# DaehwanKimLab/centrifuge

Measured on AMD Instinct MI355X. Metric: classified reads/sec (whole node) on 100bp synthetic reads vs p_compressed; HBM GB/s achieved, higher is better.
Workload: dtype u64

## Files before the change

### centrifuge_amd/csrc/cf_device.hip

```cpp
#include <hip/hip_runtime.h>
#include <sched.h>
#include <dlfcn.h>

#include <algorithm>
#include <cmath>
#include <chrono>
#include <cstdio>
#include <cstdlib>
#include <cstring>
#include <memory>
#include <mutex>
#include <stdexcept>
#include <string>
#include <vector>

#include "../../include/centrifuge_amd.h"
#include "cf_index.hpp"
#include "cf_kernels.hpp"
#include "cf_scan.hpp"
#include "cf_textio.hpp"
#include "cf_inflate.hpp"
#include "cf_restore.hpp"
#include "cf_plan.hpp"
#include "cf_knobs.hpp"
// ... 47 lines not shown
__global__ void __launch_bounds__(256) k_search(DIndex ix, DParams pr, DBatch b) { search_body<G>(ix, pr, b); }

__global__ void __launch_bounds__(256) k_rlen(const uint64_t *off, uint32_t *rlen, uint32_t nReads) { rlen_body(off, rlen, nReads, cf_global_thread()); }
__global__ void __launch_bounds__(256) k_convert(DConvert c) { convert_body(c, cf_global_thread()); }
__global__ void __launch_bounds__(256) k_dense_unpack(DUnpack u) { dense_unpack_body(u, (uint64_t)blockIdx.x * blockDim.x + threadIdx.x); }
__global__ void __launch_bounds__(256) k_pack(DBatch b, uint8_t *recs, uint32_t W) { pack_body(b, recs, W, cf_global_thread()); }

template <int G, int W, bool COUNT>
__global__ void __launch_bounds__(256) __attribute__((amdgpu_waves_per_eu(COUNT ? 1 : W == 4 ? 6 : W == 6 ? 5 : 4, 8))) k_search2(DIndex ix, DParams pr, DBatch b) {
    __shared__ __attribute__((aligned(16))) uint8_t lds[(256 / G) * rec_lds_stride(W) + 256 * 4 * RankTab<G>::WORDS + (256 / G) * 16 * kLazyHits];
    search2_body<G, W, COUNT>(ix, pr, b, lds);
}

template <int W, bool COUNT, int LZ = 0, bool MULTI = false>
__global__ void __launch_bounds__(256) __attribute__((amdgpu_waves_per_eu((W == 4 && LZ == 1) ? 7 : (W == 4 && MULTI) ? 6 : (W == 6 && MULTI) ? 5 : 1, 8))) k_search2_l1(DIndex ix, DParams pr, DBatch b) {
    __shared__ __attribute__((aligned(16))) uint8_t lds[256 * rec_lds_stride(W) + 256 * 16 * (LZ ? LZ : (int)lazy_hits(1, W))];
    search2_body<1, W, COUNT, true, LZ, MULTI>(ix, pr, b, lds);
}
__global__ void __launch_bounds__(256) k_pair_planes(DIndex ix, uint8_t *planes2, uint64_t nGroups) {
    pair_planes_body(ix, planes2, (uint64_t)blockIdx.x * blockDim.x + threadIdx.x, nGroups);
}
__global__ void __launch_bounds__(256) k_occ_planes(DIndex ix, uint8_t *planes, uint64_t nSides) {
    occ_planes_body(ix, planes, (uint64_t)blockIdx.x * blockDim.x + threadIdx.x, nSides);
}
__global__ void __launch_bounds__(256) k_repeat_probe(DIndex ix, uint32_t nSamples, uint32_t depth, uint32_t *hits) {
    const uint32_t i = cf_global_thread();
    bool yes = false;
    if (i < nSamples && ix.len > 2) {
        uint64_t x = 0x9e3779b97f4a7c15ull * (i + 1);
        x ^= x >> 29; x *= 0xbf58476d1ce4e5b9ull; x ^= x >> 32;
        yes = repeat_probe_body(ix, x % (ix.len - 1), depth);
    }
    const uint64_t m = cf_ballot(yes);
    if (m && cf_lane() == (uint32_t)cf_ctz64(m)) (void)cf_atomic_add(hits, (uint32_t)cf_popc64(m));
}

__global__ void __launch_bounds__(256) k_post_fast(DIndex ix, DParams pr, DBatch b) {
    const uint32_t q = cf_global_thread();
    const bool d = q < b.nQueries ? post_fast_body(ix, pr, b, q) : false;
    if (q < b.nQueries && b.postDeferred) b.postDeferred[q] = d ? 1 : 0;
    defer_push(b.slowPost, &b.st->nSlowPost, d, q);
}
template <bool EARLY>
__global__ void __launch_bounds__(256) k_score_fast(DIndex ix, DParams pr, DBatch b) {
    const uint32_t q = cf_global_thread();
    const bool d = q < b.nQueries ? score_fast_body<EARLY>(ix, pr, b, q) : false;
    defer_push(b.slowScore, &b.st->nSlowScore, d, q);
}
__global__ void __launch_bounds__(256) k_list_all(uint32_t *list, uint32_t *counter, uint32_t n) {
    const uint32_t q = cf_global_thread();
    if (q < n) list[q] = q;
    if (q == 0) *counter = n;
}
__global__ void __launch_bounds__(64) __attribute__((amdgpu_waves_per_eu(3, 8))) k_post(DIndex ix, DParams pr, DBatch b, uint32_t capHits) {
    extern __shared__ __attribute__((aligned(16))) uint8_t ldsPost[];
    HitP *scratch = capHits ? reinterpret_cast<HitP *>(ldsPost) + (size_t)cf_local_thread() * capHits : nullptr;
    const uint32_t n = b.st->nSlowPost;
    for (uint32_t i = cf_global_thread(); i < n; i += cf_global_threads()) post_body(ix, pr, b, b.slowPost[i], scratch, capHits);
}
__global__ void __launch_bounds__(64) k_postfix_only(DIndex ix, DParams pr, DBatch b) {
    const uint32_t i = cf_global_thread();
    if (i < b.st->nItems / 2) post_fix(ix, pr, b, b.items[i]);
}
__global__ void k_window(DBatch b, uint32_t qLo, bool keepSlow) { if (cf_global_thread() == 0) row_window_body(b, qLo, keepSlow); }
__global__ void __launch_bounds__(256) k_emit(DParams pr, DBatch b) {
    const uint32_t q = cf_global_thread();
    if (q < b.nQueries) emit_body(pr, b, q);
}
template <int G, bool COUNT>
__global__ void __launch_bounds__(256) k_walk2(DIndex ix, DBatch b) { walk2_body<G, COUNT>(ix, b); }
template <int MODE>
__global__ void __launch_bounds__(256) k_walk_table(DIndex ix, DBatch b) { walk2_body<2, false, MODE>(ix, b); }
template <typename T>
__global__ void __launch_bounds__(256) k_stop_samples(DIndex ix, T *stopVal, uint64_t *stopBits, uint64_t nSamples) {
    for (uint64_t i = (uint64_t)blockIdx.x * blockDim.x + threadIdx.x; i < nSamples; i += (uint64_t)gridDim.x * blockDim.x) {
        const uint64_t pos = trio_at(ix.saPos, i << ix.offRate);
        stopVal[pos] = static_cast<const T *>(ix.offs)[i];
        cf_atomic_or64(&stopBits[pos >> 6], 1ull << (pos & 63));
    }
}
template <typename T>
__global__ void __launch_bounds__(256) k_stop_bounds(DIndex ix, T *stopVal, uint64_t *stopBits) {
    for (uint64_t j = (uint64_t)blockIdx.x * blockDim.x + threadIdx.x; j < ix.nBound; j += (uint64_t)gridDim.x * blockDim.x) {
        const uint64_t pos = trio_at(ix.saPos, ix.boundRow[j]);
        stopVal[pos] = (T)ix.boundRef[j];
        cf_atomic_or64(&stopBits[pos >> 6], 1ull << (pos & 63));
    }
}
template <typename T>
__global__ void k_stop_end(DIndex ix, T *stopVal, uint64_t *stopBits) {
    const uint64_t pos = trio_at(ix.saPos, ix.zOff);
    stopVal[pos] = 0;
    cf_atomic_or64(&stopBits[pos >> 6], 1ull << (pos & 63));
}
template <typename T>
__global__ void __launch_bounds__(256) k_table_by_position(DIndex ix, const T *stopVal, const uint64_t *stopBits, T *table, uint64_t nRows, uint32_t *walkMax) {
    uint32_t gap = 0;
    for (uint64_t row = (uint64_t)blockIdx.x * blockDim.x + threadIdx.x; row < nRows; row += (uint64_t)gridDim.x * blockDim.x) {
        const uint64_t pos = trio_at(ix.saPos, row);
        uint64_t w = pos >> 6;
        uint64_t m = stopBits[w] & (~0ull >> (63 - (pos & 63)));
        while (m == 0 && w > 0) m = stopBits[--w];
        const uint64_t pred = m ? (w << 6) + 63 - (uint64_t)__builtin_clzll(m) : 0;
        table[row] = stopVal[pred];
        const uint32_t g = (uint32_t)(pos - pred);
        gap = g > gap ? g : gap;
    }
    for (int d = 32; d > 0; d >>= 1) { const uint32_t o = __shfl_xor(gap, d, 64); gap = o > gap ? o : gap; }
    if ((threadIdx.x & 63) == 0 && gap) atomicMax(walkMax, gap);
}
template <typename T>
// ... 1199 lines not shown
    d.recs = bt->recWords && !bt->selfRecords ? bt->recs.p : nullptr; d.recWords = bt->recWords;
    d.itemMeta = bt->selfRecords ? bt->itemMeta.p : nullptr;
}

static void enqueuePlan(cf_batch *bt, hipStream_t st) {
    const uint64_t nReads = bt->nReads;
    const DPlan &pl = bt->pl;
    HIP_OK(hipStreamWaitEvent(st, bt->ev[8], 0));
    if (bt->densePending) {
        const uint32_t L = bt->densePending - 1;
        const DUnpack u{bt->dense.p, bt->bases.p, bt->rlen.p, (uint32_t)nReads, L, bt->revDelta ? bt->bases.p + bt->revDelta : nullptr};
        bt->revMade = bt->revDelta != 0;
        const uint64_t threads = nReads * std::max<uint64_t>(((uint64_t)L + 31) >> 5, 1);
        hipLaunchKernelGGL(k_dense_unpack, dim3((unsigned)((threads + 255) / 256)), dim3(256), 0, st, u);
        bt->densePending = 0;
    }
    HIP_OK(hipEventRecord(bt->ev[5], st));
    HIP_OK(hipMemsetAsync(bt->st.p, 0, sizeof(BatchStatus), st));
    const dim3 gp((unsigned)((nReads + 1 + 255) / 256)), bl(256);
    if (bt->fromBytes && nReads) hipLaunchKernelGGL(k_rlen, gp, bl, 0, st, bt->off8.p, bt->rlen.p, (uint32_t)nReads);
    scan_enqueue<SCAN_WORDS>(bt->rlen.p, nReads, bt->woff.p, nullptr, bt->tileA.p, bt->tileC.p, st);
    if (bt->fromBytes && nReads) {
        DConvert c{bt->seq.p, bt->off8.p, bt->woff.p, bt->bases.p, bt->nmask.p, (uint32_t)nReads};
        hipLaunchKernelGGL(k_convert, dim3((unsigned)((nReads + 255) / 256)), dim3(256), 0, st, c);
    }
    if (bt->fromText && nReads) {
        const DTextPack c{bt->text.p, bt->txSeqOff.p, bt->rlen.p, bt->woff.p, bt->bases.p, bt->nmask.p, (uint32_t)nReads};
        hipLaunchKernelGGL(k_text_pack, dim3((unsigned)((nReads + 255) / 256)), dim3(256), 0, st, c);
    }
    hipLaunchKernelGGL(k_plan, gp, bl, 0, st, pl);
    scan_enqueue<SCAN_HITS>(bt->hitCap.p, nReads, bt->hitBase.p, bt->slotOf.p, bt->tileA.p, bt->tileC.p, st);
    hipLaunchKernelGGL(k_plan_fill, gp, bl, 0, st, pl);
    if (pl.revDelta && nReads && !bt->revMade) {
        const uint64_t threads = nReads * (uint64_t)bt->recWords;
        hipLaunchKernelGGL(k_rev_words, dim3((unsigned)((threads + 255) / 256)), bl, 0, st, pl, bt->recWords);
    }
    if (bt->nQueries) hipLaunchKernelGGL(k_plan_maxscore, dim3((unsigned)((bt->nQueries + 255) / 256)), bl, 0, st, bt->rlen.p, bt->pass.p,
                                         (uint32_t)bt->nQueries, bt->paired, bt->maxScore.p);
    if (bt->recWords && !bt->selfRecords && nReads) {
        const uint64_t threads = 2 * nReads * (uint64_t)bt->recWords;
        hipLaunchKernelGGL(k_pack, dim3((unsigned)((threads + 255) / 256)), bl, 0, st, bt->d, bt->recs.p, bt->recWords);
    }
    HIP_OK(hipEventRecord(bt->ev[6], st));
    bt->planned = true;
}

static dim3 listGrid(const cf_index &ix, uint64_t nq) { return dim3((unsigned)std::max<uint64_t>(1, std::min<uint64_t>((nq + 63) / 64, (uint64_t)ix.numCUs * 32))); }

static bool earlyScoreMode(const cf_batch *bt) {
    static const bool on = envInt("CF_EARLY_SCORE", 0) != 0 && envInt("CF_POST_FAST", 1) != 0 && envInt("CF_SCORE_FAST", 1) != 0 && envInt("CF_TAIL_STREAM", 0) == 0;
    return on && bt->d.directRefs != 0 && bt->tail != nullptr && bt->nQueries != 0;
}

static void enqueuePost(cf_batch *bt, hipStream_t st) {
    cf_classifier *cl = bt->cl;
    cf_index &ix = *cl->ix;
    const DBatch &d = bt->d;
    const uint32_t nq = (uint32_t)bt->nQueries;
    if (!nq) return;
    static const bool fast = envInt("CF_POST_FAST", 1) != 0;
    if (fast) hipLaunchKernelGGL(k_post_fast, dim3((nq + 255) / 256), dim3(256), 0, st, ix.d, cl->d, d);
    else hipLaunchKernelGGL(k_list_all, dim3((nq + 255) / 256), dim3(256), 0, st, bt->slowPost.p, &bt->st.p->nSlowPost, nq);
    if (earlyScoreMode(bt)) {
        HIP_OK(hipEventRecord(bt->evPostFast, st));
        HIP_OK(hipStreamWaitEvent(bt->tail, bt->evPostFast, 0));
        hipLaunchKernelGGL(k_post, listGrid(ix, nq), dim3(64), 0, bt->tail, ix.d, cl->d, d, 0u);
        HIP_OK(hipEventRecord(bt->evPost, bt->tail));
        hipLaunchKernelGGL(k_score_fast<true>, dim3((nq + 255) / 256), dim3(256), 0, st, ix.d, cl->d, d);
        HIP_OK(hipStreamWaitEvent(st, bt->evPost, 0));
        return;
    }
    static const bool postLds = envInt("CF_POST_LDS", 0) != 0;
    const uint32_t capHits = postLds ? (uint32_t)std::min<uint64_t>(60, 2 * ((uint64_t)bt->maxLenHost / (uint64_t)std::max(1, ix.h.g.ftabChars) + 2)) : 0u;
    hipLaunchKernelGGL(k_post, listGrid(ix, nq), dim3(64), (size_t)64 * capHits * sizeof(HitP), st, ix.d, cl->d, d, capHits);
}

static bool enqueueRowPass(cf_batch *bt, uint32_t qLo, hipStream_t st, bool marks, hipStream_t late = nullptr, bool early = false) {
    cf_classifier *cl = bt->cl;
    cf_index &ix = *cl->ix;
    const DBatch &d = bt->d;
    const uint32_t nq = (uint32_t)bt->nQueries;
    static const bool fast = envInt("CF_SCORE_FAST", 1) != 0;
    HIP_OK(hipMemsetAsync(bt->cursor.p + 1, 0, 8, st));
    hipLaunchKernelGGL(k_window, dim3(1), dim3(64), 0, st, d, qLo, early);
    const bool direct = d.directRefs != 0;
    if (nq && !direct) hipLaunchKernelGGL(k_emit, dim3((nq + 255) / 256), dim3(256), 0, st, cl->d, d);
    if (marks) HIP_OK(hipEventRecord(bt->ev[2], st));
    const bool counted = nq && !direct ? launchWalk(cl, bt, st) : true;
    if (marks) HIP_OK(hipEventRecord(bt->ev[3], st));
    if (nq) {
        if (early) {}
        else if (fast) hipLaunchKernelGGL(k_score_fast<false>, dim3((nq + 255) / 256), dim3(256), 0, st, ix.d, cl->d, d);
        else hipLaunchKernelGGL(k_list_all, dim3((nq + 255) / 256), dim3(256), 0, st, bt->slowScore.p, &bt->st.p->nSlowScore, nq);
        if (late && late != st) {
            HIP_OK(hipEventRecord(bt->evLate, st));
            HIP_OK(hipStreamWaitEvent(late, bt->evLate, 0));
            st = late;
        }
        if (direct) hipLaunchKernelGGL(k_resolve_slow, listGrid(ix, nq), dim3(64), 0, st, ix.d, cl->d, d);
        static const uint32_t capRows = (uint32_t)std::clamp(envInt("CF_SCORE_LDS_ROWS", 0), 0, 64), sparse = (uint32_t)std::clamp(envInt("CF_SCORE_LDS_SPARSE", 2), 1, 64);
        hipLaunchKernelGGL(k_score, listGrid(ix, nq), dim3(64), (size_t)(64 / sparse) * score_scratch_bytes(capRows), st, ix.d, cl->d, d, capRows, capRows ? sparse : 1u, 0u, 0xffffffffu);
        static const uint32_t slotBits = (uint32_t)std::clamp(envInt("CF_COUNT_SLOT_BITS", (int)kCountSlotBits), 1, (int)kCountSlotBits);
        hipLaunchKernelGGL(k_count, dim3((nq + kCountChunk - 1) / kCountChunk), dim3(1024), 0, st, d, slotBits, d.nTaxa <= (1u << slotBits));
    }
    if (marks) HIP_OK(hipEventRecord(bt->ev[4], st));
    return counted;
}

static void enqueueCompact(cf_batch *bt, hipStream_t st) {
    const uint32_t nq = (uint32_t)bt->nQueries;
    const dim3 g((nq + 1 + 255) / 256), bl(256);
    scan_enqueue<SCAN_PLAIN>(bt->nOut.p, nq, bt->rowFirst.p, nullptr, bt->tileA.p, bt->tileC.p, st);
    const bool narrow = bt->resultFormat == CF_RESULTS_NARROW;
    const DCompact c{bt->out.p, bt->o1tax.p, bt->o1a.p, bt->o1b.p, bt->d.oStride, bt->nOut.p, bt->rowFirst.p, (uint32_t)bt->cl->d.k, nq, bt->outCompact.p, bt->st.p,
                     narrow ? reinterpret_cast<NarrowRow *>(bt->outCompact.p) : nullptr, bt->qinfo.p, bt->pass.p, bt->paired};
    hipLaunchKernelGGL(k_compact, g, bl, 0, st, c);
}

static void enqueueClassify(cf_batch *bt, hipStream_t st) {
    cf_classifier *cl = bt->cl;
    HIP_OK(hipMemsetAsync(bt->cursor.p, 0, 32, st));
    HIP_OK(hipMemsetAsync(bt->ops.p, 0, sizeof(OpCounts), st));
    static const bool allFast = envInt("CF_POST_FAST", 1) != 0 && envInt("CF_SCORE_FAST", 1) != 0;
    if (!allFast) {
        HIP_OK(hipMemsetAsync(bt->qRows.p, 0, 4 * (bt->nQueries + 1), st));
        HIP_OK(hipMemsetAsync(bt->nOut.p, 0, 4 * (bt->nQueries + 1), st));
    }
// ... 1303 lines not shown
```

### centrifuge_amd/csrc/cf_kernels.hpp

```cpp
#pragma once
#include "cf_platform.hpp"

namespace cfamd {

constexpr uint32_t kNone32 = 0xffffffffu;
constexpr uint64_t kNone64 = ~0ull;
constexpr uint32_t kSideChars = 384;
constexpr int kSearchChunk = CF_WAVE;

struct RefInfo { uint64_t tax; uint32_t tidx, pid; };
static_assert(sizeof(RefInfo) == 16, "RefInfo layout");
struct DIndex {
    const uint8_t *sides;
    const uint64_t *ftab, *eftab;
    uint64_t fchr0, fchr1, fchr2, fchr3;
    uint64_t len, zOff, zSide;
    uint32_t zIn;
    int32_t ftabChars, offRate, offw;
    const void *offs;
    const uint8_t *planes;
    const uint8_t *planes2;
    const uint64_t *wide;
    int32_t wideChars;
    const uint64_t *text;
// ... 1633 lines not shown
    bool tried = false;
    uint32_t run = 0;
    while (dep < L) {
        if (ix.posRate >= 0 && !tried && bot - top == 1 && run >= ix.verifyMinRun && (top & ((1ull << ix.posRate) - 1)) == 0 &&
            L - dep >= kVerifyMinLeft) {
            tried = true;
            const uint64_t p = trio_at(ix.saPos, top >> ix.posRate);
            uint64_t tw = 0, twi = kNone64;
            uint32_t M = 0;
            while (dep + M < L && M < p) {
                const uint64_t pos = p - 1 - M;
                if ((pos >> 5) != twi) { twi = pos >> 5; tw = ix.text[twi]; }
                const int rc = strand_char(b, wbase, L, fw, L - (dep + M) - 1, win);
                if (rc > 3 || (uint64_t)rc != ((tw >> (2 * (pos & 31))) & 3)) break;
                M++;
            }
            const uint64_t pe = p - M, pm = (1ull << ix.isaRate) - 1, q = (pe + pm) & ~pm;
            if ((b.lazyHits & 4u) && (dep + M >= L || M < p)) {
                h.top = kRowIsPos | pe; h.bot = h.top + 1; h.len = dep + M - cur;
                return;
            }
            if (M >= 4 && M >= q - pe) {
                dep = dep + M - (uint32_t)(q - pe);
                top = trio_at(ix.isa, q >> ix.isaRate); bot = top + 1;
                continue;
            }
        }
        const int c = strand_char(b, wbase, L, fw, L - dep - 1, win);
        if (c > 3) break;
        uint64_t t, bb;
        { bool two; rank_any<G>(ix, c, top, bot, t, bb, two); }
        if (bb <= t) break;
        run = (bb - t == 1 && bot - top == 1) ? run + 1 : 0;
        top = t; bot = bb; dep++;
    }
    h.top = top; h.bot = bot; h.len = dep - cur;
}

CF_DEV bool hit_less(const HitP &a, const HitP &b) {
    const uint64_t as = hp_size(a), bs = hp_size(b);
    const uint64_t al = hp_len(a), bl = hp_len(b);
    if (al >= 22 || bl >= 22) {
        if (al >= 22 && bl >= 22) { if (as < bs) return true; if (as > bs) return false; }
        if (bl < al) return true;
        if (bl > al) return false;
    }
    if (bl * as < al * bs) return true;
    if (bl * as > al * bs) return false;
    if (as < bs) return true;
    if (as > bs) return false;
    if (bl < al) return true;
    return false;
}
CF_DEV void hit_swap(HitP &a, HitP &b) { const HitP t = a; a = b; b = t; }

CF_DEV void ss_linear_insert(HitP *a, int last) {
    const HitP val = a[last];
    int next = last - 1;
    while (hit_less(val, a[next])) { a[last] = a[next]; last = next; --next; }
    a[last] = val;
}
CF_DEV void ss_insertion(HitP *a, int first, int last) {
    if (first == last) return;
    for (int i = first + 1; i != last; ++i) {
        if (hit_less(a[i], a[first])) {
            const HitP val = a[i];
            for (int k = i; k > first; --k) a[k] = a[k - 1];
            a[first] = val;
        } else ss_linear_insert(a, i);
    }
}
CF_DEV void ss_push_heap(HitP *a, int first, int hole, int top, const HitP &val) {
    int parent = (hole - 1) / 2;
    while (hole > top && hit_less(a[first + parent], val)) {
        a[first + hole] = a[first + parent]; hole = parent; parent = (hole - 1) / 2;
    }
    a[first + hole] = val;
}
CF_DEV void ss_adjust_heap(HitP *a, int first, int hole, int len, const HitP &val) {
    const int top = hole;
    int child = hole;
    while (child < (len - 1) / 2) {
        child = 2 * (child + 1);
        if (hit_less(a[first + child], a[first + (child - 1)])) child--;
        a[first + hole] = a[first + child]; hole = child;
    }
    if ((len & 1) == 0 && child == (len - 2) / 2) {
        child = 2 * (child + 1);
        a[first + hole] = a[first + (child - 1)]; hole = child - 1;
    }
    ss_push_heap(a, first, hole, top, val);
}
CF_DEV void ss_heapsort(HitP *a, int first, int last) {
    const int len = last - first;
    if (len >= 2) {
        int parent = (len - 2) / 2;
        for (;;) { const HitP v = a[first + parent]; ss_adjust_heap(a, first, parent, len, v); if (parent == 0) break; parent--; }
    }
    while (last - first > 1) {
        --last;
        const HitP v = a[last]; a[last] = a[first];
        ss_adjust_heap(a, first, 0, last - first, v);
    }
}
CF_DEV void std_sort_hits(HitP *a, int n) {
    if (n <= 1) return;
    int lg = 0;
    for (int t = n; t > 1; t >>= 1) lg++;
    int stF[48], stL[48], stD[48], sp = 0;
    int first = 0, last = n, depth = 2 * lg;
    for (;;) {
        while (last - first > 16) {
            if (depth == 0) { ss_heapsort(a, first, last); break; }
            --depth;
            const int mid = first + (last - first) / 2;
            {
                const int x = first + 1, y = mid, z = last - 1;
                if (hit_less(a[x], a[y])) {
                    if (hit_less(a[y], a[z])) hit_swap(a[first], a[y]);
                    else if (hit_less(a[x], a[z])) hit_swap(a[first], a[z]);
                    else hit_swap(a[first], a[x]);
                } else if (hit_less(a[x], a[z])) hit_swap(a[first], a[x]);
                else if (hit_less(a[y], a[z])) hit_swap(a[first], a[z]);
                else hit_swap(a[first], a[y]);
            }
            int lo = first + 1, hi = last;
            for (;;) {
                while (hit_less(a[lo], a[first])) ++lo;
                --hi;
                while (hit_less(a[first], a[hi])) --hi;
                if (!(lo < hi)) break;
                hit_swap(a[lo], a[hi]);
                ++lo;
            }
            if (sp < 48) { stF[sp] = lo; stL[sp] = last; stD[sp] = depth; sp++; }
            last = lo;
        }
        if (sp == 0) break;
        --sp; first = stF[sp]; last = stL[sp]; depth = stD[sp];
    }
    if (n > 16) {
        ss_insertion(a, 0, 16);
        for (int i = 16; i != n; ++i) ss_linear_insert(a, i);
    } else ss_insertion(a, 0, n);
}

CF_DEV void hit_reset(HitP &h) { Hit z; z.top = z.bot = 0; z.bwoff = kNone32; z.len = 0; z.nelt = 0; h = hit_pack(z); }

CF_DEV void post_trim(HitP *h, uint32_t n) {
    if (n < 2) return;
    for (uint32_t i = 0; i + 1 < n; i++) {
        for (uint32_t j = i + 1; j < n; j++) {
            const uint32_t bi = hp_bwoff(h[i]), bj = hp_bwoff(h[j]), li = hp_len(h[i]), lj = hp_len(h[j]);
            if (bi >= bj) { hp_set_len(h[i], 0); break; }
            if ((uint64_t)bi + li <= bj) break;
            if (li >= lj) {
                const uint32_t e = bj + lj;
                hp_set_bwoff(h[j], bi + li); hp_set_len(h[j], e - (bi + li));
            } else hp_set_len(h[i], bj - bi);
        }
    }
}

CF_DEV void post_fix(const DIndex &ix, const DParams &pr, const DBatch &b, uint32_t rd, HitP *const hs[2], const uint32_t n[2]) {
    const uint64_t wbase = b.woff[rd], m = pr.m;
    const uint32_t L = b.rlen[rd];
    uint64_t sum[2] = {0, 0};
    for (int f = 0; f < 2; f++) for (uint32_t i = 0; i < n[f]; i++) if (hp_len(hs[f][i]) >= m) sum[f] += hp_len(hs[f][i]);
    if (sum[0] >= m && sum[1] >= m) {
        for (uint32_t i = 0; i < n[0]; i++) {
            HitP &hit = hs[0][i];
            const uint64_t len = hp_len(hit), l = hp_bwoff(hit), r = l + len;
            for (uint32_t j = 0; j < n[1]; j++) {
                HitP &rc = hs[1][j];
                const uint64_t rclen = hp_len(rc);
                if (len < m && rclen < m) continue;
                const uint64_t rc_l = (uint64_t)L - hp_bwoff(rc) - rclen, rc_r = rc_l + rclen;
                if (r <= rc_l) continue;
                if (rc_r <= l) continue;
                if (l == rc_l && r == rc_r) continue;
                if (l < rc_l && r > rc_r) continue;
                if (l > rc_l && r < rc_r) continue;
                if (l > rc_l) {
                    Hit t; ps_whole<1>(ix, b, wbase, L, true, (uint32_t)rc_l, t);
                    if (t.len == len + l - rc_l) hit = hit_pack(t);
                }
                if (r > rc_r) {
                    Hit t; ps_whole<1>(ix, b, wbase, L, false, (uint32_t)(L - r), t);
                    if (t.len == rclen + r - rc_r) rc = hit_pack(t);
                }
            }
        }
        for (uint32_t i = 0; i < n[0]; i++) {
            HitP &hit = hs[0][i];
            const uint64_t len = hp_len(hit), l = hp_bwoff(hit), r = l + len;
            for (uint32_t j = 0; j < n[1]; j++) {
                HitP &rc = hs[1][j];
                const uint64_t rclen = hp_len(rc), rc_l = (uint64_t)L - hp_bwoff(rc) - rclen, rc_r = rc_l + rclen;
                if (rc_l < l) break;
                if (len != rclen) continue;
                if (l == rc_l && r == rc_r && hp_size(hit) + hp_size(rc) > pr.ihits) {
                    hit_reset(hit); hit_reset(rc); break;
                }
            }
        }
    }
    post_trim(hs[0], n[0]);
    post_trim(hs[1], n[1]);
}
CF_DEV void post_fix(const DIndex &ix, const DParams &pr, const DBatch &b, uint32_t rd) {
    const uint32_t slot = b.slotOf[rd];
    HitP *hs[2] = {b.hits + b.hitBase[rd], b.hits + b.hitBase[rd] + b.hitCap[rd]};
    const uint32_t n[2] = {nhml_n(b.nhml[2 * slot]), nhml_n(b.nhml[2 * slot + 1])};
    post_fix(ix, pr, b, rd, hs, n);
}

CF_DEV void hits_copy(HitP *dst, const HitP *src, uint32_t n) {
    uint32_t i = 0;
    for (; i + 4 <= n; i += 4) { const HitP a = src[i], b2 = src[i + 1], c = src[i + 2], d = src[i + 3]; dst[i] = a; dst[i + 1] = b2; dst[i + 2] = c; dst[i + 3] = d; }
    for (; i < n; i++) dst[i] = src[i];
}

CF_DEV void post_body(const DIndex &ix, const DParams &pr, const DBatch &b, uint32_t q, HitP *scratch = nullptr, uint32_t scratchCap = 0) {
    if (b.st->flags & kStHitsOverflow) { b.qRows[q] = 0; return; }
    QHead qi;
    for (int a = 0; a < 2; a++) { qi.lo[a] = qi.hi[a] = 0; qi.nProc[a][0] = qi.nProc[a][1] = 0; qi.brk[a] = 0; qi.pad2[a] = 0; qi.maxG[a][0] = qi.maxG[a][1] = 0; }
    uint32_t nPlanned = 0;
    const uint32_t r0 = b.paired ? 2 * q : q;
    const bool p0 = b.pass[r0] != 0, p1 = b.paired ? b.pass[r0 + 1] != 0 : false;
    uint32_t rds[2] = {r0, r0 + 1};
    int nm;
    uint32_t isPaired = 0, firstMate = 0;
    if (b.paired && p0 && p1) { nm = 2; isPaired = 1; }
    else if (p0) nm = 1;
    else if (p1) { nm = 1; rds[0] = r0 + 1; firstMate = 1; }
    else nm = 0;
    const uint64_t k = pr.k, m = pr.m;
    uint64_t maxG = k;
    uint32_t rowsTotal = 0;
    uint32_t tsBase = 0;
    bool tsWide = false;
    for (int rdi = 0; rdi < nm; rdi++) {
        const uint32_t rd = rds[rdi], slot = b.slotOf[rd];
        HitP *const pool[2] = {b.hits + b.hitBase[rd], b.hits + b.hitBase[rd] + b.hitCap[rd]};
        HitP *hs[2] = {pool[0], pool[1]};
        const uint32_t hm0 = b.nhml[2 * slot], hm1 = b.nhml[2 * slot + 1];
        const uint32_t n[2] = {nhml_n(hm0), nhml_n(hm1)};
        const bool long0 = nhml_long(hm0), long1 = nhml_long(hm1);
        if (!long0 && !long1) continue;
        const uint32_t need = (long0 ? n[0] : 0u) + (long1 ? n[1] : 0u);
        const bool staged = scratch != nullptr && need <= scratchCap;
        if (staged) {
            hs[0] = scratch; hs[1] = scratch + (long0 ? n[0] : 0u);
            if (long0) hits_copy(hs[0], pool[0], n[0]);
            if (long1) hits_copy(hs[1], pool[1], n[1]);
        }
        if (long0 && long1) post_fix(ix, pr, b, rd, hs, n);
        else post_trim(hs[long0 ? 0 : 1], n[long0 ? 0 : 1]);
        uint64_t tot[2] = {0, 0}, mx[2] = {0, 0};
        for (int f = 0; f < 2; f++) if (f == 0 ? long0 : long1) for (uint32_t i = 0; i < n[f]; i++) {
            const uint64_t len = hp_len(hs[f][i]);
            if (len < m) continue;
            tot[f] += (len - 15) * (len - 15);
            if (len > mx[f]) mx[f] = len;
        }
        int lo, hi;
        if (tot[0] != tot[1]) { lo = tot[0] > tot[1] ? 0 : 1; hi = lo + 1; }
        else if (mx[0] != mx[1]) { lo = mx[0] > mx[1] ? 0 : 1; hi = lo + 1; }
        else { lo = 0; hi = 2; }
        qi.lo[rdi] = (uint8_t)lo; qi.hi[rdi] = (uint8_t)hi;
        for (int f = lo; f < hi; f++) {
            HitP *h = hs[f];
            for (uint32_t i = 0; i < n[f]; i++)
                if (hp_len(h[i]) >= m && hp_size(h[i]) > maxG) maxG = hp_size(h[i]);
            if (maxG > k) maxG += k;
            qi.maxG[rdi][f] = maxG > 0xffffffffull ? 0xffffffffu : (uint32_t)maxG;
            std_sort_hits(h, (int)n[f]);
            uint64_t cnt = 0;
            uint32_t i = 0;
            for (; i < n[f]; i++) {
                const uint64_t len = hp_len(h[i]), size = hp_size(h[i]);
                const uint64_t nelt = plan_nelt(len, size, maxG, m, pr.ihits);
                if (nelt == 0) continue;
                if (nPlanned < kInlinePlan) {
                    PlanHit ph;
                    ph.top = hp_row(h[i]); ph.nelt = (uint32_t)nelt; ph.meta = plan_meta((uint32_t)len, rdi, f, tsBase + i);
                    if (tsBase + i > kPlanTsMax || len > 0xffffu) tsWide = true;
                    b.qplan[(uint64_t)nPlanned * b.qplanStride + q] = ph;
                }
                nPlanned++;
                rowsTotal += (uint32_t)nelt;
                cnt += nelt;
                if (cnt >= maxG) { i++; qi.brk[rdi] |= (uint8_t)(1u << f); break; }
            }
            qi.nProc[rdi][f] = i;
            tsBase += i - ((qi.brk[rdi] >> f) & 1u);
            if (staged) hits_copy(pool[f], h, n[f]);
        }
    }
    const uint32_t nPlan = (nPlanned <= kInlinePlan && !tsWide) ? nPlanned : kPlanNotInline;
    b.qflag[q] = qf_make(nPlan, isPaired, firstMate, (uint32_t)nm);
    if (nPlan == kPlanNotInline) b.qhead[q] = qi;
    b.qRows[q] = rowsTotal;
}

CF_DEV void defer_push(uint32_t *list, uint32_t *counter, bool defer, uint32_t q) {
    const uint64_t mask = cf_ballot(defer);
    if (!mask) return;
    const uint32_t lane = cf_lane();
    const int leader = cf_ctz64(mask);
    uint32_t base = 0;
    if ((int)lane == leader) base = cf_atomic_add(counter, (uint32_t)cf_popc64(mask));
    base = cf_shfl(base, leader);
    if (defer) list[base + (uint32_t)cf_popc64(mask & ((1ull << lane) - 1))] = q;
}

constexpr int kPostFastHits = 8;
CF_DEV bool post_fast_body(const DIndex &ix, const DParams &pr, const DBatch &b, uint32_t q) {
    (void)ix;
    if (b.st->flags & kStHitsOverflow) { b.qRows[q] = 0; return false; }
    uint32_t fOf0 = 2, fOf1 = 2, np0 = 0, np1 = 0, brk0 = 0, brk1 = 0;
    uint8_t isPaired = 0, firstMate = 0;
    const uint32_t r0 = b.paired ? 2 * q : q;
    const bool p0 = b.pass[r0] != 0, p1 = b.paired ? b.pass[r0 + 1] != 0 : false;
    uint32_t rd0 = r0;
    int nm;
    if (b.paired && p0 && p1) { nm = 2; isPaired = 1; }
    else if (p0) nm = 1;
    else if (p1) { nm = 1; rd0 = r0 + 1; firstMate = 1; }
    else nm = 0;
    const uint64_t k = pr.k, m = pr.m;
    uint64_t maxG = k;
    uint32_t rowsTotal = 0, tsBase = 0, nPlanned = 0;
    PlanHit pl0{0, 0, 0}, pl1{0, 0, 0}, pl2{0, 0, 0}, pl3{0, 0, 0};
    static_assert(kInlinePlan == 4, "four plan slots below");
    bool defer = false;
    for (int rdi = 0; rdi < nm && !defer; rdi++) {
        const uint32_t rd = rd0 + (uint32_t)rdi, slot = b.slotOf[rd];
        const uint32_t hm0 = b.nhml[2 * slot], hm1 = b.nhml[2 * slot + 1];
        const bool long0 = nhml_long(hm0), long1 = nhml_long(hm1);
        if (!long0 && !long1) continue;
        if (long0 && long1) { defer = true; break; }
        const int f = long0 ? 0 : 1;
        const uint32_t n = nhml_n(f ? hm1 : hm0);
        if (n > (uint32_t)kPostFastHits) { defer = true; break; }
        const uint8_t *hp = reinterpret_cast<const uint8_t *>(b.hits + b.hitBase[rd] + (f ? b.hitCap[rd] : 0u));
        uint64_t w0[kPostFastHits], w1[kPostFastHits];
#pragma unroll
        for (int i = 0; i < kPostFastHits; i++) {
            u64x2 v{0, 0};
            if ((uint32_t)i < n) v = cf_load16(hp + 16 * i);
            w0[i] = v.x; w1[i] = v.y;
        }
        bool apart = true;
        uint64_t mg = maxG;
#pragma unroll
        for (int i = 0; i < kPostFastHits; i++) {
// ... 879 lines not shown
```

Baseline: 1.429 billion.

## Split slow post kernel into paired extension and planning kernels with LDS sort stack

Replaces the monolithic slow post kernel with two kernels. The first runs the forward/reverse hit extension with two lanes per query, splitting the ps_whole calls across lanes and exchanging results via lane swaps. The second does the strand weighting, sorting and planning, with the quicksort stack moved from private arrays into LDS and packed into 64-bit entries. It also smallest-partition-first recursion to bound stack depth, and the QHead struct is built from scalars to cut register and stack pressure. The aim is less scratch spilling and better parallelism on the divergent slow path, at the cost of an extra kernel launch, an extra pass over the hits in global memory, and dropping the optional LDS hit staging.

```diff
diff --git a/centrifuge_amd/csrc/cf_device.hip b/centrifuge_amd/csrc/cf_device.hip
--- a/centrifuge_amd/csrc/cf_device.hip
+++ b/centrifuge_amd/csrc/cf_device.hip
@@ -123,11 +123,11 @@
     if (q < n) list[q] = q;
     if (q == 0) *counter = n;
 }
-__global__ void __launch_bounds__(64) __attribute__((amdgpu_waves_per_eu(3, 8))) k_post(DIndex ix, DParams pr, DBatch b, uint32_t capHits) {
-    extern __shared__ __attribute__((aligned(16))) uint8_t ldsPost[];
-    HitP *scratch = capHits ? reinterpret_cast<HitP *>(ldsPost) + (size_t)cf_local_thread() * capHits : nullptr;
+__global__ void __launch_bounds__(64) k_post_ext(DIndex ix, DParams pr, DBatch b) { post_ext_list<2>(ix, pr, b, cf_global_thread(), cf_global_threads()); }
+__global__ void __launch_bounds__(64) k_post_plan(DParams pr, DBatch b) {
+    __shared__ uint64_t sortStack[kSortStack * 64];
     const uint32_t n = b.st->nSlowPost;
-    for (uint32_t i = cf_global_thread(); i < n; i += cf_global_threads()) post_body(ix, pr, b, b.slowPost[i], scratch, capHits);
+    for (uint32_t i = cf_global_thread(); i < n; i += cf_global_threads()) post_plan_body(pr, b, b.slowPost[i], sortStack + cf_local_thread(), 64u);
 }
 __global__ void __launch_bounds__(64) k_postfix_only(DIndex ix, DParams pr, DBatch b) {
     const uint32_t i = cf_global_thread();
@@ -1433,6 +1433,14 @@
     return on && bt->d.directRefs != 0 && bt->tail != nullptr && bt->nQueries != 0;
 }
 
+static void enqueuePostGeneral(cf_batch *bt, hipStream_t st) {
+    cf_classifier *cl = bt->cl;
+    cf_index &ix = *cl->ix;
+    const uint64_t nq = bt->nQueries;
+    hipLaunchKernelGGL(k_post_ext, listGrid(ix, 2 * nq), dim3(64), 0, st, ix.d, cl->d, bt->d);
+    hipLaunchKernelGGL(k_post_plan, listGrid(ix, nq), dim3(64), 0, st, cl->d, bt->d);
+}
+
 static void enqueuePost(cf_batch *bt, hipStream_t st) {
     cf_classifier *cl = bt->cl;
     cf_index &ix = *cl->ix;
@@ -1445,15 +1453,13 @@
     if (earlyScoreMode(bt)) {
         HIP_OK(hipEventRecord(bt->evPostFast, st));
         HIP_OK(hipStreamWaitEvent(bt->tail, bt->evPostFast, 0));
-        hipLaunchKernelGGL(k_post, listGrid(ix, nq), dim3(64), 0, bt->tail, ix.d, cl->d, d, 0u);
+        enqueuePostGeneral(bt, bt->tail);
         HIP_OK(hipEventRecord(bt->evPost, bt->tail));
         hipLaunchKernelGGL(k_score_fast<true>, dim3((nq + 255) / 256), dim3(256), 0, st, ix.d, cl->d, d);
         HIP_OK(hipStreamWaitEvent(st, bt->evPost, 0));
         return;
     }
-    static const bool postLds = envInt("CF_POST_LDS", 0) != 0;
-    const uint32_t capHits = postLds ? (uint32_t)std::min<uint64_t>(60, 2 * ((uint64_t)bt->maxLenHost / (uint64_t)std::max(1, ix.h.g.ftabChars) + 2)) : 0u;
-    hipLaunchKernelGGL(k_post, listGrid(ix, nq), dim3(64), (size_t)64 * capHits * sizeof(HitP), st, ix.d, cl->d, d, capHits);
+    enqueuePostGeneral(bt, st);
 }
 
 static bool enqueueRowPass(cf_batch *bt, uint32_t qLo, hipStream_t st, bool marks, hipStream_t late = nullptr, bool early = false) {
diff --git a/centrifuge_amd/csrc/cf_kernels.hpp b/centrifuge_amd/csrc/cf_kernels.hpp
--- a/centrifuge_amd/csrc/cf_kernels.hpp
+++ b/centrifuge_amd/csrc/cf_kernels.hpp
@@ -1709,10 +1709,11 @@
     if (bl < al) return true;
     return false;
 }
-CF_DEV void hit_swap(HitP &a, HitP &b) { const HitP t = a; a = b; b = t; }
+CF_DEV HitP hp_copy(const HitP &p) { HitP r; r.w0 = p.w0; r.w1 = p.w1; return r; }
+CF_DEV void hit_swap(HitP &a, HitP &b) { const HitP t = hp_copy(a); a = hp_copy(b); b = t; }
 
 CF_DEV void ss_linear_insert(HitP *a, int last) {
-    const HitP val = a[last];
+    const HitP val = hp_copy(a[last]);
     int next = last - 1;
     while (hit_less(val, a[next])) { a[last] = a[next]; last = next; --next; }
     a[last] = val;
@@ -1721,8 +1722,8 @@
     if (first == last) return;
     for (int i = first + 1; i != last; ++i) {
         if (hit_less(a[i], a[first])) {
-            const HitP val = a[i];
-            for (int k = i; k > first; --k) a[k] = a[k - 1];
+            const HitP val = hp_copy(a[i]);
+            for (int k = i; k > first; --k) a[k] = hp_copy(a[k - 1]);
             a[first] = val;
         } else ss_linear_insert(a, i);
     }
@@ -1752,19 +1753,20 @@
     const int len = last - first;
     if (len >= 2) {
         int parent = (len - 2) / 2;
-        for (;;) { const HitP v = a[first + parent]; ss_adjust_heap(a, first, parent, len, v); if (parent == 0) break; parent--; }
+        for (;;) { const HitP v = hp_copy(a[first + parent]); ss_adjust_heap(a, first, parent, len, v); if (parent == 0) break; parent--; }
     }
     while (last - first > 1) {
         --last;
-        const HitP v = a[last]; a[last] = a[first];
+        const HitP v = hp_copy(a[last]); a[last] = hp_copy(a[first]);
         ss_adjust_heap(a, first, 0, last - first, v);
     }
 }
-CF_DEV void std_sort_hits(HitP *a, int n) {
+constexpr int kSortStack = 24;
+CF_DEV void std_sort_hits(HitP *a, int n, uint64_t *st, uint32_t stStride) {
     if (n <= 1) return;
     int lg = 0;
     for (int t = n; t > 1; t >>= 1) lg++;
-    int stF[48], stL[48], stD[48], sp = 0;
+    int sp = 0;
     int first = 0, last = n, depth = 2 * lg;
     for (;;) {
         while (last - first > 16) {
@@ -1790,11 +1792,15 @@
                 hit_swap(a[lo], a[hi]);
                 ++lo;
             }
-            if (sp < 48) { stF[sp] = lo; stL[sp] = last; stD[sp] = depth; sp++; }
-            last = lo;
+            const bool leftSmall = lo - first <= last - lo;
+            const int wf = leftSmall ? lo : first, wl = leftSmall ? last : lo;
+            if (wl - wf > 16 && sp < kSortStack) { st[(uint32_t)sp * stStride] = (uint64_t)wf | ((uint64_t)wl << 28) | ((uint64_t)depth << 56); sp++; }
+            if (leftSmall) last = lo; else first = lo;
         }
         if (sp == 0) break;
-        --sp; first = stF[sp]; last = stL[sp]; depth = stD[sp];
+        --sp;
+        const uint64_t e = st[(uint32_t)sp * stStride];
+        first = (int)(e & 0xfffffffu); last = (int)((e >> 28) & 0xfffffffu); depth = (int)(e >> 56);
     }
     if (n > 16) {
         ss_insertion(a, 0, 16);
@@ -1819,40 +1825,67 @@
     }
 }
 
-CF_DEV void post_fix(const DIndex &ix, const DParams &pr, const DBatch &b, uint32_t rd, HitP *const hs[2], const uint32_t n[2]) {
+template <int PAIR>
+CF_DEV void post_fix(const DIndex &ix, const DParams &pr, const DBatch &b, uint32_t rd, HitP *h0, HitP *h1, uint32_t n0, uint32_t n1, uint32_t sub) {
     const uint64_t wbase = b.woff[rd], m = pr.m;
     const uint32_t L = b.rlen[rd];
-    uint64_t sum[2] = {0, 0};
-    for (int f = 0; f < 2; f++) for (uint32_t i = 0; i < n[f]; i++) if (hp_len(hs[f][i]) >= m) sum[f] += hp_len(hs[f][i]);
-    if (sum[0] >= m && sum[1] >= m) {
-        for (uint32_t i = 0; i < n[0]; i++) {
-            HitP &hit = hs[0][i];
+    uint32_t both = 0;
+    if (sub == 0) {
+        uint64_t sum0 = 0, sum1 = 0;
+        for (uint32_t i = 0; i < n0; i++) { const uint64_t len = hp_len(h0[i]); if (len >= m) sum0 += len; }
+        for (uint32_t i = 0; i < n1; i++) { const uint64_t len = hp_len(h1[i]); if (len >= m) sum1 += len; }
+        both = sum0 >= m && sum1 >= m ? 1u : 0u;
+    }
+    if (PAIR == 2) { const uint32_t o = cf_swap1(both); if (sub) both = o; }
+    if (both) {
+        for (uint32_t i = 0; i < n0; i++) {
+            uint64_t len = 0, l = 0, r = 0;
+            if (sub == 0) { const HitP hit = h0[i]; len = hp_len(hit); l = hp_bwoff(hit); r = l + len; }
+            for (uint32_t j = 0; j < n1; j++) {
+                uint64_t rclen = 0, rc_l = 0, rc_r = 0;
+                uint32_t due = 0;
+                if (sub == 0) {
+                    const HitP rc = h1[j];
+                    rclen = hp_len(rc);
+                    rc_l = (uint64_t)L - hp_bwoff(rc) - rclen; rc_r = rc_l + rclen;
+                    const bool skip = (len < m && rclen < m) || r <= rc_l || rc_r <= l || (l == rc_l && r == rc_r) ||
+                                      (l < rc_l && r > rc_r) || (l > rc_l && r < rc_r);
+                    if (!skip) due = (l > rc_l ? 1u : 0u) | (r > rc_r ? 2u : 0u);
+                }
+                if (PAIR == 2) {
+                    const uint32_t order = cf_swap1(sub == 0 && due == 3 ? 0x80000000u | (uint32_t)((uint64_t)L - r) : 0u);
+                    const bool mine = sub == 0 ? due != 0 : (order >> 31) != 0;
+                    const bool two = sub == 0 ? due == 3 : mine;
+                    const bool fw = sub == 0 && (due & 1u) != 0;
+                    const uint32_t cur = sub ? order & 0x7fffffffu : fw ? (uint32_t)rc_l : (uint32_t)((uint64_t)L - r);
+                    HitP mineP{0, 0};
+                    if (mine) { Hit t; ps_whole<1>(ix, b, wbase, L, fw, cur, t); mineP = hit_pack(t); }
+                    HitP secondP = mineP;
+                    if (two) {
+                        secondP.w0 = (uint64_t)cf_swap1((uint32_t)mineP.w0) | ((uint64_t)cf_swap1((uint32_t)(mineP.w0 >> 32)) << 32);
+                        secondP.w1 = (uint64_t)cf_swap1((uint32_t)mineP.w1) | ((uint64_t)cf_swap1((uint32_t)(mineP.w1 >> 32)) << 32);
+                    }
+                    if (sub == 0) {
+                        if ((due & 1u) && hp_len(mineP) == len + l - rc_l) h0[i] = mineP;
+                        if ((due & 2u) && hp_len(secondP) == rclen + r - rc_r) h1[j] = secondP;
+                    }
+                } else {
+                    if (due & 1u) {
+                        Hit t; ps_whole<1>(ix, b, wbase, L, true, (uint32_t)rc_l, t);
+                        if (t.len == len + l - rc_l) h0[i] = hit_pack(t);
+                    }
+                    if (due & 2u) {
+                        Hit t; ps_whole<1>(ix, b, wbase, L, false, (uint32_t)(L - r), t);
+                        if (t.len == rclen + r - rc_r) h1[j] = hit_pack(t);
+                    }
+                }
+            }
+        }
+        if (sub == 0) for (uint32_t i = 0; i < n0; i++) {
+            HitP &hit = h0[i];
             const uint64_t len = hp_len(hit), l = hp_bwoff(hit), r = l + len;
-            for (uint32_t j = 0; j < n[1]; j++) {
-                HitP &rc = hs[1][j];
-                const uint64_t rclen = hp_len(rc);
-                if (len < m && rclen < m) continue;
-                const uint64_t rc_l = (uint64_t)L - hp_bwoff(rc) - rclen, rc_r = rc_l + rclen;
-                if (r <= rc_l) continue;
-                if (rc_r <= l) continue;
-                if (l == rc_l && r == rc_r) continue;
-                if (l < rc_l && r > rc_r) continue;
-                if (l > rc_l && r < rc_r) continue;
-                if (l > rc_l) {
-                    Hit t; ps_whole<1>(ix, b, wbase, L, true, (uint32_t)rc_l, t);
-                    if (t.len == len + l - rc_l) hit = hit_pack(t);
-                }
-                if (r > rc_r) {
-                    Hit t; ps_whole<1>(ix, b, wbase, L, false, (uint32_t)(L - r), t);
-                    if (t.len == rclen + r - rc_r) rc = hit_pack(t);
-                }
-            }
-        }
-        for (uint32_t i = 0; i < n[0]; i++) {
-            HitP &hit = hs[0][i];
-            const uint64_t len = hp_len(hit), l = hp_bwoff(hit), r = l + len;
-            for (uint32_t j = 0; j < n[1]; j++) {
-                HitP &rc = hs[1][j];
+            for (uint32_t j = 0; j < n1; j++) {
+                HitP &rc = h1[j];
                 const uint64_t rclen = hp_len(rc), rc_l = (uint64_t)L - hp_bwoff(rc) - rclen, rc_r = rc_l + rclen;
                 if (rc_l < l) break;
                 if (len != rclen) continue;
@@ -1862,80 +1895,89 @@
             }
         }
     }
-    post_trim(hs[0], n[0]);
-    post_trim(hs[1], n[1]);
+    if (sub == 0) { post_trim(h0, n0); post_trim(h1, n1); }
 }
 CF_DEV void post_fix(const DIndex &ix, const DParams &pr, const DBatch &b, uint32_t rd) {
     const uint32_t slot = b.slotOf[rd];
-    HitP *hs[2] = {b.hits + b.hitBase[rd], b.hits + b.hitBase[rd] + b.hitCap[rd]};
-    const uint32_t n[2] = {nhml_n(b.nhml[2 * slot]), nhml_n(b.nhml[2 * slot + 1])};
-    post_fix(ix, pr, b, rd, hs, n);
-}
-
-CF_DEV void hits_copy(HitP *dst, const HitP *src, uint32_t n) {
-    uint32_t i = 0;
-    for (; i + 4 <= n; i += 4) { const HitP a = src[i], b2 = src[i + 1], c = src[i + 2], d = src[i + 3]; dst[i] = a; dst[i + 1] = b2; dst[i + 2] = c; dst[i + 3] = d; }
-    for (; i < n; i++) dst[i] = src[i];
-}
-
-CF_DEV void post_body(const DIndex &ix, const DParams &pr, const DBatch &b, uint32_t q, HitP *scratch = nullptr, uint32_t scratchCap = 0) {
-    if (b.st->flags & kStHitsOverflow) { b.qRows[q] = 0; return; }
-    QHead qi;
-    for (int a = 0; a < 2; a++) { qi.lo[a] = qi.hi[a] = 0; qi.nProc[a][0] = qi.nProc[a][1] = 0; qi.brk[a] = 0; qi.pad2[a] = 0; qi.maxG[a][0] = qi.maxG[a][1] = 0; }
-    uint32_t nPlanned = 0;
+    post_fix<1>(ix, pr, b, rd, b.hits + b.hitBase[rd], b.hits + b.hitBase[rd] + b.hitCap[rd], nhml_n(b.nhml[2 * slot]), nhml_n(b.nhml[2 * slot + 1]), 0u);
+}
+
+CF_DEV int post_mates(const DBatch &b, uint32_t q, uint32_t &rd0, uint32_t &isPaired, uint32_t &firstMate) {
     const uint32_t r0 = b.paired ? 2 * q : q;
     const bool p0 = b.pass[r0] != 0, p1 = b.paired ? b.pass[r0 + 1] != 0 : false;
-    uint32_t rds[2] = {r0, r0 + 1};
-    int nm;
-    uint32_t isPaired = 0, firstMate = 0;
-    if (b.paired && p0 && p1) { nm = 2; isPaired = 1; }
-    else if (p0) nm = 1;
-    else if (p1) { nm = 1; rds[0] = r0 + 1; firstMate = 1; }
-    else nm = 0;
+    const bool both = p0 && p1, second = !p0 && p1;
+    rd0 = r0 + (second ? 1u : 0u); isPaired = both ? 1u : 0u; firstMate = second ? 1u : 0u;
+    return both ? 2 : (p0 || p1) ? 1 : 0;
+}
+
+template <int PAIR>
+CF_DEV void post_ext_body(const DIndex &ix, const DParams &pr, const DBatch &b, uint32_t q, uint32_t sub) {
+    if (b.st->flags & kStHitsOverflow) return;
+    uint32_t rd0, isPaired, firstMate;
+    const int nm = post_mates(b, q, rd0, isPaired, firstMate);
+    for (int rdi = 0; rdi < nm; rdi++) {
+        const uint32_t rd = rd0 + (uint32_t)rdi, slot = b.slotOf[rd];
+        HitP *const h0 = b.hits + b.hitBase[rd], *const h1 = h0 + b.hitCap[rd];
+        const uint32_t hm0 = b.nhml[2 * slot], hm1 = b.nhml[2 * slot + 1];
+        const bool long0 = nhml_long(hm0), long1 = nhml_long(hm1);
+        if (long0 && long1) post_fix<PAIR>(ix, pr, b, rd, h0, h1, nhml_n(hm0), nhml_n(hm1), sub);
+        else if (sub == 0 && long0) post_trim(h0, nhml_n(hm0));
+        else if (sub == 0 && long1) post_trim(h1, nhml_n(hm1));
+    }
+}
+template <int PAIR>
+CF_DEV void post_ext_list(const DIndex &ix, const DParams &pr, const DBatch &b, uint32_t thread, uint32_t threads) {
+    const uint32_t n = b.st->nSlowPost;
+    for (uint32_t i = thread / PAIR; i < n; i += threads / PAIR) post_ext_body<PAIR>(ix, pr, b, b.slowPost[i], PAIR == 2 ? thread & 1u : 0u);
+}
+
+CF_DEV void post_strand_weight(const HitP *h, uint32_t n, uint64_t m, uint64_t &tot, uint64_t &mx) {
+    for (uint32_t i = 0; i < n; i++) {
+        const uint64_t len = hp_len(h[i]);
+        if (len < m) continue;
+        tot += (len - 15) * (len - 15);
+        if (len > mx) mx = len;
+    }
+}
+
+CF_DEV void post_plan_body(const DParams &pr, const DBatch &b, uint32_t q, uint64_t *sortStack, uint32_t sortStride) {
+    if (b.st->flags & kStHitsOverflow) { b.qRows[q] = 0; return; }
+    uint32_t np00 = 0, np01 = 0, np10 = 0, np11 = 0, mg00 = 0, mg01 = 0, mg10 = 0, mg11 = 0;
+    uint32_t lo0 = 0, lo1 = 0, hi0 = 0, hi1 = 0, brk0 = 0, brk1 = 0;
+    uint32_t nPlanned = 0;
+    uint32_t rd0, isPaired, firstMate;
+    const int nm = post_mates(b, q, rd0, isPaired, firstMate);
     const uint64_t k = pr.k, m = pr.m;
     uint64_t maxG = k;
     uint32_t rowsTotal = 0;
     uint32_t tsBase = 0;
     bool tsWide = false;
     for (int rdi = 0; rdi < nm; rdi++) {
-        const uint32_t rd = rds[rdi], slot = b.slotOf[rd];
-        HitP *const pool[2] = {b.hits + b.hitBase[rd], b.hits + b.hitBase[rd] + b.hitCap[rd]};
-        HitP *hs[2] = {pool[0], pool[1]};
+        const uint32_t rd = rd0 + (uint32_t)rdi, slot = b.slotOf[rd];
+        HitP *const h0 = b.hits + b.hitBase[rd], *const h1 = h0 + b.hitCap[rd];
         const uint32_t hm0 = b.nhml[2 * slot], hm1 = b.nhml[2 * slot + 1];
-        const uint32_t n[2] = {nhml_n(hm0), nhml_n(hm1)};
+        const uint32_t n0 = nhml_n(hm0), n1 = nhml_n(hm1);
         const bool long0 = nhml_long(hm0), long1 = nhml_long(hm1);
         if (!long0 && !long1) continue;
-        const uint32_t need = (long0 ? n[0] : 0u) + (long1 ? n[1] : 0u);
-        const bool staged = scratch != nullptr && need <= scratchCap;
-        if (staged) {
-            hs[0] = scratch; hs[1] = scratch + (long0 ? n[0] : 0u);
-            if (long0) hits_copy(hs[0], pool[0], n[0]);
-            if (long1) hits_copy(hs[1], pool[1], n[1]);
-        }
-        if (long0 && long1) post_fix(ix, pr, b, rd, hs, n);
-        else post_trim(hs[long0 ? 0 : 1], n[long0 ? 0 : 1]);
-        uint64_t tot[2] = {0, 0}, mx[2] = {0, 0};
-        for (int f = 0; f < 2; f++) if (f == 0 ? long0 : long1) for (uint32_t i = 0; i < n[f]; i++) {
-            const uint64_t len = hp_len(hs[f][i]);
-            if (len < m) continue;
-            tot[f] += (len - 15) * (len - 15);
-            if (len > mx[f]) mx[f] = len;
-        }
+        uint64_t tot0 = 0, tot1 = 0, mx0 = 0, mx1 = 0;
+        if (long0) post_strand_weight(h0, n0, m, tot0, mx0);
+        if (long1) post_strand_weight(h1, n1, m, tot1, mx1);
         int lo, hi;
-        if (tot[0] != tot[1]) { lo = tot[0] > tot[1] ? 0 : 1; hi = lo + 1; }
-        else if (mx[0] != mx[1]) { lo = mx[0] > mx[1] ? 0 : 1; hi = lo + 1; }
+        if (tot0 != tot1) { lo = tot0 > tot1 ? 0 : 1; hi = lo + 1; }
+        else if (mx0 != mx1) { lo = mx0 > mx1 ? 0 : 1; hi = lo + 1; }
         else { lo = 0; hi = 2; }
-        qi.lo[rdi] = (uint8_t)lo; qi.hi[rdi] = (uint8_t)hi;
+        if (rdi) { lo1 = (uint32_t)lo; hi1 = (uint32_t)hi; } else { lo0 = (uint32_t)lo; hi0 = (uint32_t)hi; }
         for (int f = lo; f < hi; f++) {
-            HitP *h = hs[f];
-            for (uint32_t i = 0; i < n[f]; i++)
+            HitP *h = f ? h1 : h0;
+            const uint32_t nf = f ? n1 : n0;
+            for (uint32_t i = 0; i < nf; i++)
                 if (hp_len(h[i]) >= m && hp_size(h[i]) > maxG) maxG = hp_size(h[i]);
             if (maxG > k) maxG += k;
-            qi.maxG[rdi][f] = maxG > 0xffffffffull ? 0xffffffffu : (uint32_t)maxG;
-            std_sort_hits(h, (int)n[f]);
+            const uint32_t mg = maxG > 0xffffffffull ? 0xffffffffu : (uint32_t)maxG;
+            std_sort_hits(h, (int)nf, sortStack, sortStride);
             uint64_t cnt = 0;
-            uint32_t i = 0;
-            for (; i < n[f]; i++) {
+            uint32_t i = 0, brk = 0;
+            for (; i < nf; i++) {
                 const uint64_t len = hp_len(h[i]), size = hp_size(h[i]);
                 const uint64_t nelt = plan_nelt(len, size, maxG, m, pr.ihits);
                 if (nelt == 0) continue;
@@ -1948,18 +1990,38 @@
                 nPlanned++;
                 rowsTotal += (uint32_t)nelt;
                 cnt += nelt;
-                if (cnt >= maxG) { i++; qi.brk[rdi] |= (uint8_t)(1u << f); break; }
-            }
-            qi.nProc[rdi][f] = i;
-            tsBase += i - ((qi.brk[rdi] >> f) & 1u);
-            if (staged) hits_copy(pool[f], h, n[f]);
+                if (cnt >= maxG) { i++; brk = 1; break; }
+            }
+            if (rdi) { if (f) { np11 = i; mg11 = mg; } else { np10 = i; mg10 = mg; } brk1 |= brk << f; }
+            else { if (f) { np01 = i; mg01 = mg; } else { np00 = i; mg00 = mg; } brk0 |= brk << f; }
+            tsBase += i - brk;
         }
     }
     const uint32_t nPlan = (nPlanned <= kInlinePlan && !tsWide) ? nPlanned : kPlanNotInline;
     b.qflag[q] = qf_make(nPlan, isPaired, firstMate, (uint32_t)nm);
-    if (nPlan == kPlanNotInline) b.qhead[q] = qi;
+    if (nPlan == kPlanNotInline) {
+        QHead qi;
+        qi.nProc[0][0] = np00; qi.nProc[0][1] = np01; qi.nProc[1][0] = np10; qi.nProc[1][1] = np11;
+        qi.lo[0] = (uint8_t)lo0; qi.lo[1] = (uint8_t)lo1; qi.hi[0] = (uint8_t)hi0; qi.hi[1] = (uint8_t)hi1;
+        qi.brk[0] = (uint8_t)brk0; qi.brk[1] = (uint8_t)brk1; qi.pad2[0] = qi.pad2[1] = 0;
+        qi.maxG[0][0] = mg00; qi.maxG[0][1] = mg01; qi.maxG[1][0] = mg10; qi.maxG[1][1] = mg11;
+        b.qhead[q] = qi;
+    }
     b.qRows[q] = rowsTotal;
 }
+
+#ifdef CF_HOST_EMU
+inline void std_sort_hits(HitP *a, int n) { uint64_t st[kSortStack]; std_sort_hits(a, n, st, 1); }
+#ifdef CF_EMU_OWN_POST_BODY
+void post_body(const DIndex &ix, const DParams &pr, const DBatch &b, uint32_t q, HitP *scratch, uint32_t cap);
+#else
+inline void post_body(const DIndex &ix, const DParams &pr, const DBatch &b, uint32_t q, HitP *, uint32_t) {
+    uint64_t st[kSortStack];
+    post_ext_body<1>(ix, pr, b, q, 0);
+    post_plan_body(pr, b, q, st, 1);
+}
+#endif
+#endif
 
 CF_DEV void defer_push(uint32_t *list, uint32_t *counter, bool defer, uint32_t q) {
     const uint64_t mask = cf_ballot(defer);
```

Result: no change. 1.441 billion (median of 6 runs) (+0.8%).
